# DanielQ-51/cudapathtracer

Measured on AMD Instinct MI355X. Metric: Mray/s, higher is better.
Workload: dtype f32; 1 GPU; cornell_1920x1080_1024spp_depth8_mis; spp=1024, max_depth=8, integrator=UNIDIRECTIONAL (MIS), variant=megakernel, seed=103033, triangles=36, bvh_nodes=31

## Files before the change

### cudapathtracer_amd/csrc/pt_megakernel.h

```cpp
#pragma once
#include "pt_path.h"
#include "pt_params.h"

namespace pt {

PT_DEV void wave_add_total(unsigned long long* totals, int k, uint32_t v) {
    unsigned long long s = v;
    for (int off = 32; off > 0; off >>= 1) s += __shfl_down(s, off, 64);
    if ((threadIdx.x & 63) == 0 && s) atomicAdd(&totals[k], s);
}

extern __shared__ __attribute__((aligned(16))) unsigned char pt_smem[];

PT_DEV SceneCache stage_scene_cache(const DeviceScene& S, int cacheNodes, int cacheTris, int attrOff = 0, int nA = 0, int nM = 0, int nL = 0) {
    typedef __attribute__((address_space(3))) f4v lds_f4;
    lds_f4* dstN = (lds_f4*)pt_smem;
    lds_f4* dstT = dstN + cacheNodes * 4;
    const f4v* srcN = reinterpret_cast<const f4v*>(S.nodes);
    const f4v* srcT = reinterpret_cast<const f4v*>(S.tris);
    for (int i = threadIdx.x; i < cacheNodes * 4; i += blockDim.x) dstN[i] = srcN[i];
    for (int i = threadIdx.x; i < cacheTris * 3; i += blockDim.x) dstT[i] = srcT[i];
    if (attrOff > 0) {
        lds_f4* dA = (lds_f4*)(pt_smem + attrOff);
        lds_f4* dM = dA + nA * 5;
// ... 252 lines not shown
            PT_STAMP(2);
            const int nBusy = __builtin_popcountll(__ballot((rs.flags & kRayBusy) != 0));
            if (nBusy == 0) break;
            trace_resume<COUNT, STACKN, ONCHIP, NOLEAF, TRISEL>(S, SC, st, rs, ps.o, ps.d, (nBusy * P.refillKeep) >> 4, thr, h, c, Keep{P.nodeKeep, P.triKeep});
            PT_STAMP(1);
            continue;
        }
#ifdef PT_STAMPS
        occ[0] += 64; occ[1] += __builtin_popcountll(__ballot((ps.flags & kInPath) != 0 || (samplesLeft > 0 && !stopStarting)));
#endif
        const uint32_t flagsIn = ps.flags;
        if (DEFER) apply_pending<NOLEAF, ARMS>(ps, thr, acc);
        if constexpr (MOMENTS && DEFER) landed_by_apply(flagsIn);
        if (ps.flags & kInPath) {
            bool done = path_bounce<INTEG, COUNT, DEFER, SIMPLE, LEAN, NOLEAF, LTRI, ARMS>(S, ps, ms, h, P.maxDepth, P.useMIS, shadowSync, c, LTRI ? P.lightTri8 : 0ull);
            if (!done) done = path_exhausted<INTEG>(ps, P.maxDepth);
            if (done) { path_finish(ps, acc, DEFER); if constexpr (MOMENTS) landed_by_finish(); }
        }
        PT_STAMP(2);
        while (!(ps.flags & kInPath) && samplesLeft > 0 && !stopStarting) {
            samplesLeft--;
            path_begin<COUNT, ARMS>(P.cam, ps, ms, PT_PX, PT_PY, c);
            if (path_exhausted<INTEG>(ps, P.maxDepth)) { path_finish(ps, acc, DEFER); if constexpr (MOMENTS) landed_by_finish(); }
        }
        if constexpr (ARMS) { if (ps.flags & kDirRaw) ps.d = normalize(ps.d); }
        const bool hasExt = (ps.flags & kInPath) != 0;
        const bool hasShadow = DEFER && (ps.flags & kShadowPending) != 0;
        PT_STAMP(0);
#ifdef PT_STAMPS
        occ[2] += __builtin_popcountll(__ballot(hasExt)); occ[3] += __builtin_popcountll(__ballot(hasShadow));
#endif
        if (__ballot(hasExt || hasShadow) == 0ull) break;
        if constexpr (DEFER && FLAT) {
            trace_pair_flat<STACKN, ARMS>(S, SC, st, hasShadow, ps.so, ps.sd, ps.smaxt, LTRI ? (ps.flags & kLightTriMask) >> kLightTriShift : 0u, hasExt, ps.o, ps.d, thr, h, c, P.cacheNodes, P.leaves, P.nLeaves);
        }
        else if constexpr (FLAT) {
            trace_closest_flat<STACKN, FLATW>(S, SC, hasExt, ps.o, ps.d, 999999.0f, st, h, c, P.cacheNodes, P.leaves, P.nLeaves);
        }
        else if (hasExt) trace_closest<COUNT, STACKN, ONCHIP, CULL>(S, SC, ps.o, ps.d, 999999.0f, st, h, c, Keep{P.nodeKeep, P.triKeep});
        PT_STAMP(1);
    }

    if (lpt) {
        if (lane == 0) { atomicAdd(&P.queue[4], -myRem); atomicAdd(&P.queue[5], -1); }
        __builtin_amdgcn_s_setprio(0);
    }
#ifdef PT_STAMPS
    if (P.totals && lane == 0) {
        for (int k = 0; k < 3; k++) atomicAdd(&P.totals[8 + k], stamp[k]);
        atomicAdd(&P.totals[14], stamp[3]);
        const unsigned long long wall1 = wall_clock64();
        atomicAdd(&P.totals[11], wall1 - wall0);
        atomicMax(&P.totals[12], ~wall0);
        atomicMax(&P.totals[13], wall1);
        if (!COUNT) {
            atomicAdd(&P.totals[0], occ[2]); atomicAdd(&P.totals[1], occ[3]);
            atomicAdd(&P.totals[7], occ[1]); atomicAdd(&P.totals[15], occ[0]);
        }
    }
#endif
    if (inImage) {
        uint32_t* o = (uint32_t*)(P.out + (size_t)lt * 64 + lane);
        state_store(o, __float_as_uint(acc.x), shared); state_store(o + 1, __float_as_uint(acc.y), shared);
        state_store(o + 2, __float_as_uint(acc.z), shared);
    }
    {
        uint32_t* r = P.rng + (size_t)lt * 384 + lane;
// ... 88 lines not shown
```

### cudapathtracer_amd/csrc/pt_plan.h

```cpp
#pragma once
#include "pt_params.h"

namespace pt {

struct Options {
    int variant = 0;
    int cull = 0;
    int schedMask = 31;
    int sliceAlways = 1;
    int sliceIters = 512;
    int lptPrio = 2;
    int persistent = 1;
    int queueTimeoutMs = 30000;
    int onchipOk = 1;
    bool wavesHbmOk = true;
    bool wavesHbmForce = false;
    int nodeKeep = 10, triKeep = 8;
    int refill = 1, refillKeep = 6;
    bool refillKeepSet = false;
    int flatWanted = 1, simpleWanted = 1, leanWanted = 1;
    int leafBoxes = 1;
    int flat2Wanted = 1;
    int wfWideWg = 1;
    int momentsFused = 0;
};
struct Facts {
    DeviceScene ds{};
    int stackNeed = 0, nInternal = 0, cacheNodes = 0, cacheTris = 0, nTrisPacked = 0, nMats = 0, nLightsPacked = 0;
    int nLeaves = 0;
    unsigned long long lightTri8 = 0ull;
    bool armless = false;
    bool noLeafTris = false;
    bool simpleOk = false;
    bool leanOk = false;
    bool flatOk = false;
};

int scene_onchip_wg(const Facts& F, const Options& O);
bool scene_onchip(const Facts& F, const Options& O);
bool hbm_kernel_pays(const Facts& F, const Options& O, int numCU, bool simple, long long tiles);

struct LaunchAsk { int integrator; bool count; int useMIS; int live; };
struct LaunchPlan {
    int onchipWg;
    bool hbm, cull, refill;
    int flat;
    bool simple, lean;
    bool simpleTimed, timedHbm;
};
LaunchPlan plan_launch(const Facts& F, const Options& O, int numCU, const LaunchAsk& ask);
KParams plan_selectors(const LaunchPlan& plan);

struct LaunchSizes { int spillEntries, blocks, queueCap; };
LaunchSizes size_launch(const Facts& F, const Options& O, int numCU, const LaunchAsk& ask, const TileSpan& t, bool listed,
                        const LaunchPlan& plan, const MkRow& row, KParams& P);

}
```

### cudapathtracer_amd/csrc/pt_plan.hip

```cpp
#include <algorithm>

#include "../../include/pt_api.h"
#include "pt_plan.h"

namespace pt {

int scene_onchip_wg(const Facts& F, const Options& O) {
    if (!O.onchipOk || F.nTrisPacked <= 0 || F.ds.stackSpill != 0) return 0;
    const size_t geom = (size_t)F.nInternal * 64 + (size_t)F.nTrisPacked * 48, rec = attr_cache_bytes(F.nTrisPacked, F.nMats, F.nLightsPacked);
    const size_t perWave = (size_t)kStackFlat2Rows * 256 + (F.simpleOk && O.simpleWanted ? 0 : (size_t)kMediumMax * 64);
    for (int wg = 4; wg <= 16; wg *= 2)
        if (geom <= (size_t)kCacheBytes * (wg / 4) && (kAttrCacheBytes == 0 || rec <= (size_t)kAttrCacheBytes * (wg / 4)) &&
            geom + rec + (size_t)wg * perWave <= (size_t)160 * 1024 * wg / 16) return wg;
    return 0;
}
bool scene_onchip(const Facts& F, const Options& O) { return scene_onchip_wg(F, O) > 0; }
bool hbm_kernel_pays(const Facts& F, const Options& O, int numCU, bool simple, long long tiles) {
    if (scene_onchip(F, O) || !O.wavesHbmOk) return false;
    const long long slots = (long long)numCU * 4 * (simple ? kWavesHbmSimple : kWavesHbm);
    return O.wavesHbmForce || tiles * 4 >= slots * (simple ? 3 : 5);
}

LaunchPlan plan_launch(const Facts& F, const Options& O, int numCU, const LaunchAsk& ask) {
    LaunchPlan p = {};
// ... 14 lines not shown
    p.lean = F.leanOk && O.leanWanted && !F.armless && !p.simple && !ask.count && !p.cull && (p.flat == 3 || (!onchip && p.refill));
    return p;
}

KParams plan_selectors(const LaunchPlan& plan) {
    KParams P = {};
    P.onchip = plan.onchipWg > 0 ? 1 : 0;
    P.hbm = plan.hbm ? 1 : 0;
    P.cull = plan.cull ? 1 : 0;
    P.refill = plan.refill ? 1 : 0;
    P.flat = plan.flat;
    P.simple = plan.simple ? 1 : 0;
    P.lean = plan.lean ? 1 : 0;
    return P;
}

LaunchSizes size_launch(const Facts& F, const Options& O, int numCU, const LaunchAsk& ask, const TileSpan& t, bool listed,
                        const LaunchPlan& plan, const MkRow& row, KParams& P) {
    const bool onchip = plan.onchipWg > 0;
    LaunchSizes z = {};
    z.spillEntries = plan.hbm ? std::max(0, F.stackNeed - row.f.stackEntries) : F.ds.stackSpill;
    P.wgWaves = row.f.wgWaves ? row.f.wgWaves : (onchip ? plan.onchipWg : 4);
    P.wavesPerSimd = row.f.wavesPerSimd;
    z.blocks = megakernel_blocks(t.count, P.wgWaves);
    P.S = F.ds;
    P.S.stackSpill = z.spillEntries;
    P.useMIS = ask.useMIS;
    P.tileFirst = t.first; P.tileStride = t.stride; P.tileCount = t.count; P.tilesX = t.tilesX;
    P.cacheNodes = F.cacheNodes; P.cacheTris = F.cacheTris;
    P.lightTri8 = F.lightTri8;
    if (onchip) { P.cacheNodes = F.nInternal; P.cacheTris = F.nTrisPacked; }
    if (onchip && kAttrCacheBytes > 0) { P.cacheAttrs = F.nTrisPacked; P.cacheMats = F.nMats; P.cacheLights = F.nLightsPacked; }
    if (onchip && kAttrCacheBytes > 0 && F.flatOk && O.leafBoxes && F.nLeaves > 0) P.nLeaves = F.nLeaves;
    if (plan.hbm && F.cacheTris == 0) P.cacheNodes = std::min(F.nInternal, (plan.simple ? kCacheBytesHbmSimple : kCacheBytesHbm) / 64);
    P.gnodeFrom = P.cacheNodes;
    if (ask.count && !onchip && F.cacheTris == 0) {
        P.gnodeFrom = plan.timedHbm ? std::min(F.nInternal, (plan.simpleTimed ? kCacheBytesHbmSimple : kCacheBytesHbm) / 64) : F.cacheNodes;
    }
    P.refillKeep = (plan.hbm || O.refillKeepSet) ? O.refillKeep : kRefillKeepSmall;
    P.nodeKeep = O.nodeKeep; P.triKeep = O.triKeep;
    P.lptPrio = O.lptPrio; P.sliceIters = O.sliceIters; P.schedMask = O.schedMask; P.sliceAlways = O.sliceAlways ? 1 : 0;
    P.queueTimeout = (unsigned long long)O.queueTimeoutMs * 100000ull;
    if (O.persistent || listed) {
        z.queueCap = 256;
        while (z.queueCap < t.count) z.queueCap <<= 1;
        P.queueMask = z.queueCap - 1;
        P.gridBlocks = numCU * P.wavesPerSimd * 4 / P.wgWaves;
    }
    return z;
}

}
```

### cudapathtracer_amd/csrc/pt_render.hip

```cpp
#include "pt_host.h"

using namespace pt;

namespace pt {

int resolve_tiles(int w, int h, const pt_tile_range* tiles, TileSpan& t) {
    if (w <= 0 || h <= 0) return fail(-1, "bad image size %dx%d", w, h);
    t.tilesX = (w + 7) / 8;
    int total = t.tilesX * ((h + 7) / 8);
    if (!tiles) { t.first = 0; t.stride = 1; t.count = total; return 0; }
    t.first = tiles->first; t.stride = tiles->stride; t.count = tiles->count;
    if (t.count < 0 || t.stride < 1 || t.first < 0) return fail(-1, "bad tile range {first %d, stride %d, count %d}", t.first, t.stride, t.count);
    if (t.count > 0 && (long long)t.first + (long long)(t.count - 1) * t.stride >= total)
        return fail(-1, "tile range {first %d, stride %d, count %d} exceeds the %d tiles of a %dx%d image", t.first, t.stride, t.count, total, w, h);
    return 0;
}

CamK cam_to_kernel(const pt_camera& c) {
    CamK k;
    k.origin = V3{c.cameraOrigin.x, c.cameraOrigin.y, c.cameraOrigin.z};
    k.forward = V3{c.forward.x, c.forward.y, c.forward.z};
    k.right = V3{c.right.x, c.right.y, c.right.z};
    k.up = V3{c.up.x, c.up.y, c.up.z};
    k.w = c.w; k.h = c.h; k.aperture = c.aperture; k.focalDist = c.focalDist; k.fovScale = c.fovScale; k.jitter = c.antiAliasJitterDist;
// ... 78 lines not shown
    HIP_OK(hipEventRecord(s->dev.ev1, rq.stream));
    s->last.evPending = true;
    return 0;
}

static int render_tiles(pt_scene* s, RenderRequest& rq) {
    const TileSpan& t = rq.t;
    if (t.count == 0) return 0;
    if (rq.fused && s->opt.variant == 1) return 0;
    const int live = rq.list ? rq.live : t.count;
    if (rq.list && (rq.count || s->opt.variant != 0 || t.first != 0 || t.stride != 1 || live < 0 || live > t.count)) return fail(-1, "render_tiles: bad tile list");
    if (int r = s->work.rng.ensure((size_t)t.count * 384 * sizeof(uint32_t))) return r;
    if (!rq.continueStreams) HIP_OK(launch_rng_init((const uint32_t*)s->data.jump.p, rq.seed, rq.w, rq.h, t, (uint32_t*)s->work.rng.p, rq.stream));
    if (rq.fused) rq.seeded = !rq.continueStreams;
    if (s->opt.variant == 1) return render_tiles_wavefront(s, rq);

    const LaunchAsk ask = {rq.integrator, rq.count, rq.useMIS, live};
    const LaunchPlan plan = plan_launch(s->facts, s->opt, s->dev.numCU, ask);
    KParams P = plan_selectors(plan);
    const MkRow* row = megakernel_choose(rq.integrator, rq.count, true, P, false);
    if (!row) return fail(-1, "render_tiles: no megakernel is built for this launch");
    const LaunchSizes z = size_launch(s->facts, s->opt, s->dev.numCU, ask, t, rq.list != nullptr, plan, *row, P);

    if (z.spillEntries > 0)
        if (int r = s->work.spill.ensure((size_t)z.blocks * P.wgWaves * z.spillEntries * 64 * sizeof(int32_t))) return r;
    if (z.queueCap > 0) {
        if (int r = s->work.queue.ensure((size_t)(kQueueHeader + 2 * z.queueCap) * sizeof(int))) return r;
        if (int r = s->work.left.ensure((size_t)t.count * 64 * sizeof(int))) return r;
        P.queue = (int*)s->work.queue.p; P.left = (int*)s->work.left.p;
    }
    P.cam = cam_to_kernel(*rq.cam);
    P.w = rq.w; P.h = rq.h; P.spp = rq.spp; P.maxDepth = rq.maxDepth;
    if (P.nLeaves > 0) P.leaves = (const PLeaf*)s->geo.leaves.p;
    P.rng = (uint32_t*)s->work.rng.p; P.out = (float4*)rq.d_tiles; P.pixCounters = rq.d_pixcnt;
    P.totals = rq.count ? (unsigned long long*)s->data.totals.p : nullptr;
#ifdef PT_STAMPS
    P.totals = (unsigned long long*)s->data.totals.p;
#endif
    P.spill = z.spillEntries > 0 ? (int32_t*)s->work.spill.p : nullptr;

    s->last.lean = P.lean; s->last.refill = P.refill; s->last.hbm = P.hbm;
    s->last.flat = (P.flat && !rq.count) ? 1 : 0;
    s->last.simple = (P.simple && !rq.count) ? 1 : 0;
    s->last.flat2 = (P.flat == 3) ? 1 : 0;
    s->last.leafTable = (P.flat && !rq.count && P.nLeaves > 0) ? 1 : 0;
    s->last.queued = P.queue != nullptr;
    s->last.tiles = t.count;
    s->last.pushed = live;

    MomentsK M = {nullptr, nullptr, 0, 0.0f};
    if (rq.fused) {
        row = megakernel_choose(rq.integrator, rq.count, true, P, true);
        if (!row || (row->key & kMkBuiltOnly)) return 0;
        M.P = rq.P; M.Q = rq.Q; M.c = rq.c; M.rc = 1.0f / (float)rq.c;
        rq.launched = true;
    }
    HIP_OK(hipEventRecord(s->dev.ev0, rq.stream));
    HIP_OK(launch_megakernel(*row, P, live, rq.list, rq.stream, rq.fused ? &M : nullptr));
    HIP_OK(hipEventRecord(s->dev.ev1, rq.stream));
    s->last.evPending = true;
    return 0;
}

int pt_render_tiles_device(pt_scene* s, const pt_camera* cam, int w, int h, int spp, int maxDepth, int integrator, int useMIS,
                           uint64_t seed, const pt_tile_range* tiles, void* d_tile_rgba, int count_work, void* stream) {
    if (int r = check_render_args(s, cam, spp, integrator)) return r;
// ... 355 lines not shown
```

### cudapathtracer_amd/csrc/pt_scene.hip

```cpp
#include <chrono>
#include <cmath>

#include "pt_host.h"
#include "pt_bvh_build.h"
#include "xorwow_host.h"

using namespace pt;

static_assert(sizeof(pt_bvh_node) == 48 && sizeof(pt_triangle) == 80 && sizeof(pt_material) == 176 && sizeof(pt_camera) == 112,
              "boundary structs must keep the reference's CUDA layouts (SURVEY.md Appendix A)");
static_assert(offsetof(pt_triangle, emission) == 48 && offsetof(pt_triangle, lightInd) == 64, "Triangle layout");
static_assert(offsetof(pt_material, type) == 32 && offsetof(pt_material, albedo) == 48 && offsetof(pt_material, eta) == 80 &&
              offsetof(pt_material, ior) == 112 && offsetof(pt_material, isSpecular) == 128 && offsetof(pt_material, absorption) == 144 &&
              offsetof(pt_material, priority) == 160, "Material layout");
static_assert(offsetof(pt_camera, forward) == 64 && offsetof(pt_camera, fovScale) == 44, "Camera layout");

static double wall_ms() { return std::chrono::duration<double, std::milli>(std::chrono::steady_clock::now().time_since_epoch()).count(); }

static int upload(DevBuf& b, const void* src, size_t bytes) {
    if (int r = b.ensure(std::max<size_t>(bytes, 16))) return r;
    if (bytes) HIP_OK(hipMemcpy(b.p, src, bytes, hipMemcpyHostToDevice));
    return 0;
}

static bool boxes_nested_and_finite(const std::vector<PNode>& pn, int nInternal) {
    for (int i = 0; i < nInternal; i++) {
        const PNode& p = pn[i];
        for (int a = 0; a < 3; a++)
            if (!(std::isfinite(p.lmin[a]) && std::isfinite(p.lmax[a]) && std::isfinite(p.rmin[a]) && std::isfinite(p.rmax[a]))) return false;
        const int32_t ref[2] = {p.left, p.right};
        for (int k = 0; k < 2; k++) {
            if (ref[k] < 0) continue;
            if (ref[k] <= i || ref[k] >= nInternal) return false;
            const PNode& c = pn[ref[k]];
            const float* mn = k == 0 ? p.lmin : p.rmin; const float* mx = k == 0 ? p.lmax : p.rmax;
            for (int a = 0; a < 3; a++)
                if (!(mn[a] <= c.lmin[a] && mn[a] <= c.rmin[a] && mx[a] >= c.lmax[a] && mx[a] >= c.rmax[a])) return false;
        }
    }
    return true;
}

template <class LightIndOf>
static void light_triangles(const PTri* pt, int nT, const PLight* lights, int nLights, int nTriangles, LightIndOf lightIndOf, int32_t* out) {
    for (int i = 0; i < nLights; i++) {
        out[i] = -1;
        const PLight& L = lights[i];
        const float v0[3] = {L.a[0], L.a[1], L.a[2]}, e1[3] = {L.b[0] - L.a[0], L.b[1] - L.a[1], L.b[2] - L.a[2]},
                    e2[3] = {L.c[0] - L.a[0], L.c[1] - L.a[1], L.c[2] - L.a[2]};
        for (int p = 0; p < nT && p < 63; p++) {
            const int idx = (int)(pt[p].idx & 0x7fffffffu);
            if (idx >= nTriangles || lightIndOf(idx) != i) continue;
            if (!memcmp(pt[p].v0, v0, 12) && !memcmp(pt[p].e1, e1, 12) && !memcmp(pt[p].e2, e2, 12)) { out[i] = p; break; }
        }
    }
}
static void light_triangles(const PTri* pt, int nT, const pt_scene_desc* d, int32_t* out) {
    std::vector<PLight> L((size_t)std::max(d->n_lights, 1));
    std::vector<uint8_t> bad((size_t)std::max(d->n_lights, 1), 0);
    for (int i = 0; i < d->n_lights; i++) {
        const pt_triangle& t = d->lights[i];
        L[i] = PLight{};
        if (t.aInd < 0 || t.aInd >= d->n_positions || t.bInd < 0 || t.bInd >= d->n_positions || t.cInd < 0 || t.cInd >= d->n_positions) { bad[i] = 1; continue; }
        const pt_float4 a = d->positions[t.aInd], b = d->positions[t.bInd], c = d->positions[t.cInd];
        L[i].a[0] = a.x; L[i].a[1] = a.y; L[i].a[2] = a.z; L[i].b[0] = b.x; L[i].b[1] = b.y; L[i].b[2] = b.z; L[i].c[0] = c.x; L[i].c[1] = c.y; L[i].c[2] = c.z;
    }
    light_triangles(pt, nT, L.data(), d->n_lights, d->n_triangles, [&](int idx) { const int li = d->triangles[idx].lightInd; return (li >= 0 && li < d->n_lights && bad[li]) ? -1 : li; }, out);
}

static int pack_materials(const pt_material* materials, int nMats, int nTexels, const char* fn, std::vector<PMat>& mats, std::vector<uint32_t>& matClass) {
    mats.resize((size_t)nMats); matClass.resize((size_t)nMats);
    std::memset(mats.data(), 0, mats.size() * sizeof(PMat));
    for (int i = 0; i < nMats; i++) {
// ... 83 lines not shown
    if ((size_t)nInternal * 64 + (size_t)nT * 48 <= (size_t)kCacheBytes) { s->facts.cacheNodes = nInternal; s->facts.cacheTris = nT; }
    else { s->facts.cacheNodes = std::min(nInternal, kCacheBytes / 64); s->facts.cacheTris = 0; }
    s->facts.flatOk = false;
    if (nInternal <= 128 && nT >= 1 && nT <= 128 && scene_onchip_wg(s->facts, s->opt) > 0) {
        std::vector<PNode> pn((size_t)std::max(nInternal, 1));
        std::vector<PTri> pt((size_t)nT);
        if (nInternal > 0) HIP_OK(hipMemcpy(pn.data(), s->geo.nodes.p, (size_t)nInternal * sizeof(PNode), hipMemcpyDeviceToHost));
        HIP_OK(hipMemcpy(pt.data(), s->geo.tris.p, (size_t)nT * sizeof(PTri), hipMemcpyDeviceToHost));
        auto leafCount = [&](int first) {
            int k = first;
            while (k < nT) { uint32_t w; memcpy(&w, (const char*)&pt[k] + 36, 4); k++; if (w & 0x80000000u) return k - first; }
            return 0;
        };
        bool ok = rootRef < 0 ? (~rootRef == 0 && leafCount(0) == nT) : (rootRef == 0);
        std::vector<int> first((size_t)std::max(nInternal, 1), 0);
        for (int i = nInternal - 1; i >= 0 && ok; i--) {
            int32_t* ref = &pn[i].left;
            int firstOf[2] = {0, 0};
            for (int k = 0; k < 2 && ok; k++) {
                if (ref[k] >= 0) {
                    ok = ref[k] > i && ref[k] < nInternal;
                    if (ok) { ref[2 + k] = pn[ref[k]].pad0 + pn[ref[k]].pad1; firstOf[k] = first[ref[k]]; }
                } else {
                    const int f = ~ref[k]; const int cnt = (ref[k] != kRefNone && f < nT) ? leafCount(f) : 0;
                    ok = cnt >= 1; ref[2 + k] = cnt; firstOf[k] = f;
                }
            }
            ok = ok && firstOf[1] == firstOf[0] + ref[2];
            first[i] = firstOf[0];
        }
        if (ok && nInternal > 0) ok = first[0] == 0 && pn[0].pad0 + pn[0].pad1 == nT;
        if (ok && nInternal > 0) HIP_OK(hipMemcpy(s->geo.nodes.p, pn.data(), (size_t)nInternal * sizeof(PNode), hipMemcpyHostToDevice));
        s->facts.flatOk = ok;
        s->facts.nLeaves = 0;
        if (ok && nLights > 0 && haveLights) {
            light_triangles(pt.data(), nT, hostLights, nLights, nLightInd, [&](int idx) { return lightIndOf[idx]; }, lightTri.data());
            for (int i = 0; i < nLights && i < 8; i++) s->facts.lightTri8 |= (uint64_t)(lightTri[i] + 1) << (8 * i);
        }
        if (ok && nInternal > 0 && boxes_nested_and_finite(pn, nInternal)) {
            std::vector<PLeaf> lf;
            for (int i = 0; i < nInternal; i++) {
                const int32_t* ref = &pn[i].left;
                for (int k = 0; k < 2; k++) {
                    if (ref[k] >= 0) continue;
                    PLeaf L;
                    const float* mn = k == 0 ? pn[i].lmin : pn[i].rmin; const float* mx = k == 0 ? pn[i].lmax : pn[i].rmax;
                    for (int a = 0; a < 3; a++) { L.mn[a] = mn[a]; L.mx[a] = mx[a]; }
                    L.first = ~ref[k]; L.count = ref[2 + k];
                    lf.push_back(L);
                }
            }
            if (int r = upload(s->geo.leaves, lf.data(), lf.size() * sizeof(PLeaf))) return r;
            s->facts.nLeaves = (int)lf.size();
        }
    }
    return 0;
}

static pt_float4 pos(const pt_scene_desc* d, int i, const char* what, int tri, bool& ok) {
    if (i < 0 || i >= d->n_positions) { ok = false; fail(-1, "pt_scene_create: triangle %d %s index %d out of range", tri, what, i); return pt_float4{0, 0, 0, 0}; }
    return d->positions[i];
}

static int number_nodes(const pt_bvh_node* bvh, int nN, int nT, std::vector<PNode>& nodes, std::vector<uint8_t>& leafEnd, int& nInternal, int& rootRef) {
    std::vector<int> internalId(nN, -1);
    for (int i = 0; i < nN; i++) {
        const pt_bvh_node& n = bvh[i];
        if (n.primCount > 0) {
            if (n.first < 0 || n.first + n.primCount > nT) return fail(-1, "pt_scene_create: leaf %d range [%d,+%d) out of bounds", i, n.first, n.primCount);
        } else {
            if (n.left < 0 || n.right < 0 || n.left >= nN || n.right >= nN) return fail(-1, "pt_scene_create: internal node %d has child out of range", i);
        }
    }
    {
        std::vector<int> queue;
        if (bvh[0].primCount <= 0) { queue.push_back(0); internalId[0] = nInternal++; }
        for (size_t q = 0; q < queue.size(); q++) {
            const pt_bvh_node& n = bvh[queue[q]];
            for (int c : {n.left, n.right}) {
                if (bvh[c].primCount > 0) continue;
                if (internalId[c] >= 0 || (int)queue.size() >= nN) return fail(-1, "pt_scene_create: BVH is not a tree");
                internalId[c] = nInternal++;
                queue.push_back(c);
            }
        }
    }
// ... 449 lines not shown
```

### cudapathtracer_amd/csrc/pt_trace.h

```cpp
#pragma once
#include "pt_device.h"

namespace pt {

struct Ctr {
    uint32_t raysClosest, raysShadow, pops, boxes, tris, hits, draws, iters;
    uint32_t gnodes;
    uint32_t gnodeFrom;
#ifdef PT_UTIL
    uint32_t u[8];
#endif
};
#ifdef PT_UTIL
#define PT_UTIL_STEP(c, k) do { if (COUNT) { (c).u[(k) + 1]++; const uint64_t e_ = __builtin_amdgcn_ballot_w64(true); \
    if (__builtin_amdgcn_mbcnt_hi((uint32_t)(e_ >> 32), __builtin_amdgcn_mbcnt_lo((uint32_t)e_, 0u)) == 0u) (c).u[k]++; } } while (0)
#else
#define PT_UTIL_STEP(c, k) do {} while (0)
#endif

typedef float f4v __attribute__((ext_vector_type(4)));
PT_DEV int32_t f2i(float f) { return __builtin_bit_cast(int32_t, f); }
PT_DEV uint32_t f2u(float f) { return __builtin_bit_cast(uint32_t, f); }
typedef __attribute__((address_space(3))) int32_t lds_i32;
typedef __attribute__((address_space(3))) const f4v lds_cf4;
// ... 142 lines not shown
    return n;
}
struct TriData { f4v a, b, e; };
template <bool ONCHIP = false>
PT_DEV TriData load_tri(const DeviceScene& S, const SceneCache& C, int32_t i) {
    TriData t;
    if (ONCHIP || C.nTris) {
        lds_cf4* p = C.tris + i * 3;
        t.a = p[0]; t.b = p[1]; t.e = p[2];
    } else {
        const f4v* p = reinterpret_cast<const f4v*>(S.tris + i);
        t.a = p[0]; t.b = p[1]; t.e = p[2];
    }
    return t;
}

struct TriEdges { f4v a, b; float e2z; };
PT_DEV TriEdges load_tri_edges(const SceneCache& C, int32_t i) {
    TriEdges t;
    lds_cf4* p = C.tris + i * 3;
    t.a = p[0]; t.b = p[1];
    t.e2z = *reinterpret_cast<__attribute__((address_space(3))) const float*>(p + 2);
    return t;
}
struct LeafBox { float mnx, mny, mnz, mxx, mxy, mxz; int32_t first, count; };
PT_DEV LeafBox leaf_box(const PLeaf* __restrict__ leaves, int k) {
    typedef __attribute__((address_space(4))) const float konst_f;
    typedef __attribute__((address_space(4))) const int32_t konst_i;
    konst_f* p = (konst_f*)(uintptr_t)(leaves + k);
    LeafBox L;
    L.mnx = p[0]; L.mny = p[1]; L.mnz = p[2]; L.mxx = p[3]; L.mxy = p[4]; L.mxz = p[5];
    L.first = ((konst_i*)p)[6]; L.count = ((konst_i*)p)[7];
    return L;
}

struct Keep { int node, tri; };
PT_DEV int lanes_here() { return __builtin_popcountll(__builtin_amdgcn_ballot_w64(true)); }

template <bool COUNT, int N, bool ONCHIP = false, bool CULL = false>
PT_DEV int32_t descend_node(const NodeData& n, int32_t cur, V3 o, V3 inv, Stack<N>& st, Ctr& c, float cullT = 0.0f);

template <bool COUNT, int N, bool ONCHIP = false, bool CULL = false>
PT_DEV int32_t descend(const DeviceScene& S, const SceneCache& C, int32_t cur, V3 o, V3 inv, Stack<N>& st, Ctr& c, float cullT = 0.0f) {
    const NodeData n = load_node<ONCHIP>(S, C, cur);
    return descend_node<COUNT, N, ONCHIP, CULL>(n, cur, o, inv, st, c, cullT);
}

template <bool COUNT, int N, bool ONCHIP, bool CULL>
PT_DEV int32_t descend_node(const NodeData& n, int32_t cur, V3 o, V3 inv, Stack<N>& st, Ctr& c, float cullT) {
    if (COUNT) { c.pops++; c.boxes += 2; if (!ONCHIP && (uint32_t)cur >= c.gnodeFrom) c.gnodes++; }
    float tL, tR;
    bool hL = slab(n.a.x, n.a.y, n.a.z, n.a.w, n.b.x, n.b.y, o, inv, tL);
    bool hR = slab(n.b.z, n.b.w, n.c.x, n.c.y, n.c.z, n.c.w, o, inv, tR);
    if (CULL) { hL = hL && !(tL > cullT); hR = hR && !(tR > cullT); }
    int32_t left = f2i(n.d.x), right = f2i(n.d.y);
    if (!ONCHIP && !COUNT && !CULL && N == 16) {
        if (__builtin_expect(__builtin_amdgcn_ballot_w64(st.sp >= N - 1) == 0ull, 1)) {
            if (hL && hR) {
                bool leftNear = tL < tR;
                st.template push<true>(leftNear ? right : left);
                return leftNear ? left : right;
            }
            if (hL) return left;
            if (hR) return right;
            return st.sp > 0 ? st.template pop<true>() : kRefNone;
        }
// ... 360 lines not shown
                }
                int32_t ref = S.rootRef;
                int lo = 0;
                while (ref >= 0) {
                    const NodeData nd = load_node<true>(S, C, ref);
                    const int mid = lo + f2i(nd.d.z), hi = mid + f2i(nd.d.w);
                    const Set inL = tied & Set::range(lo, mid - lo), inR = tied & Set::range(mid, hi - mid);
                    bool goLeft = !inR.any();
                    if (inL.any() && inR.any()) {
                        float tL, tR;
                        slab(nd.a.x, nd.a.y, nd.a.z, nd.a.w, nd.b.x, nd.b.y, o, inv, tL);
                        slab(nd.b.z, nd.b.w, nd.c.x, nd.c.y, nd.c.z, nd.c.w, o, inv, tR);
                        goLeft = tL < tR;
                    }
                    ref = goLeft ? f2i(nd.d.x) : f2i(nd.d.y);
                    if (!goLeft) lo = mid;
                    tied = goLeft ? inL : inR;
                }
                win = tied.first();
            }
            const TriData q = load_tri<true>(S, C, win);
            float t, u, v;
            moller_trumbore(v3(q.a.x, q.a.y, q.a.z), v3(q.a.w, q.b.x, q.b.y), v3(q.b.z, q.b.w, q.e.x), o, d, t, u, v);
            hit.t = t; hit.u = u; hit.v = v;
            hit.tri = (int32_t)(f2u(q.e.y) & 0x7fffffffu);
            hit.material = f2i(q.e.z);
        }
    }
    wave_lds_sync();
}

template <int N, bool ARMS = false>
PT_DEV void trace_pair_flat(const DeviceScene& S, const SceneCache& C, Stack<N>& st, bool hasShadow, V3 so, V3 sd, float smaxt, uint32_t ltri1,
                            bool hasExt, V3 eo, V3 ed, V3& thr, Hit& hit, Ctr& c, int nInternal, const PLeaf* __restrict__ leaves = nullptr, int nLeaves = 0) {
    static_assert(N >= 24, "the scratch layout needs 24 x 64 words of the wave's stack area");
    typedef __attribute__((address_space(3))) unsigned long long lds_u64;
    const int lane = (int)(threadIdx.x & 63u);
    lds_i32* Wd = st.lds - lane;
    typedef __attribute__((address_space(3))) f4v lds_f4;
    constexpr int kMax = 8 * 128, kKeyA = ARMS ? 8 * 128 : 9 * 128, kKeyB = kKeyA + 256, kPre = kKeyA;
    static_assert(kKeyB + (ARMS ? 256 : 128) == 24 * 64 && (ARMS || kMax + 128 == kKeyA), "records, (bounds,) first minima, second minima: 24 rows of 64 words");
    lds_f4* Rec = (lds_f4*)Wd;
    V3 invE, invS;
    if constexpr (ARMS) { invE = inv3_uniform(ed, hasExt); invS = inv3_uniform(sd, hasShadow); }
    else { invE = inv3(ed); invS = inv3(sd); }
    uint64_t tmE = 0ull, tmS = 0ull;
    if (S.rootRef < 0) { const uint64_t all = ~0ull >> (64 - S.nTris); tmE = hasExt ? all : 0ull; tmS = hasShadow ? all : 0ull; }
    else if (nLeaves > 0 && __builtin_amdgcn_ballot_w64((hasExt && !inv_is_regular(invE)) || (hasShadow && !inv_is_regular(invS))) == 0ull) {
        _Pragma("unroll 2")
        for (int k = 0; k < nLeaves; ++k) {
            const LeafBox L = leaf_box(leaves, k);
            const bool eH = slab_hit(L.mnx, L.mny, L.mnz, L.mxx, L.mxy, L.mxz, eo, invE);
            const bool sH = slab_hit(L.mnx, L.mny, L.mnz, L.mxx, L.mxy, L.mxz, so, invS);
            const uint64_t m = ((1ull << (uint32_t)L.count) - 1ull) << (uint32_t)L.first;
            tmE |= eH ? m : 0ull; tmS |= sH ? m : 0ull;
        }
        tmE = hasExt ? tmE : 0ull; tmS = hasShadow ? tmS : 0ull;
    } else {
        uint64_t visE = hasExt ? 1ull << (uint32_t)S.rootRef : 0ull, visS = hasShadow ? 1ull << (uint32_t)S.rootRef : 0ull;
        for (int i = 0; i < nInternal; ++i) {
            const bool vE = ((visE >> i) & 1ull) != 0ull, vS = ((visS >> i) & 1ull) != 0ull;
            if (__builtin_amdgcn_ballot_w64(vE || vS) == 0ull) continue;
            const NodeData n = load_node<true>(S, C, i);
            float t0, t1;
            const bool eL = slab(n.a.x, n.a.y, n.a.z, n.a.w, n.b.x, n.b.y, eo, invE, t0) && vE;
            const bool eR = slab(n.b.z, n.b.w, n.c.x, n.c.y, n.c.z, n.c.w, eo, invE, t1) && vE;
            const bool sL = slab(n.a.x, n.a.y, n.a.z, n.a.w, n.b.x, n.b.y, so, invS, t0) && vS;
            const bool sR = slab(n.b.z, n.b.w, n.c.x, n.c.y, n.c.z, n.c.w, so, invS, t1) && vS;
            const int32_t left = __builtin_amdgcn_readfirstlane(f2i(n.d.x)), right = __builtin_amdgcn_readfirstlane(f2i(n.d.y));
            const int32_t cntL = __builtin_amdgcn_readfirstlane(f2i(n.d.z)), cntR = __builtin_amdgcn_readfirstlane(f2i(n.d.w));
            const uint64_t bL = left >= 0 ? 1ull << (uint32_t)left : (~0ull >> (64 - cntL)) << (uint32_t)(~left);
            const uint64_t bR = right >= 0 ? 1ull << (uint32_t)right : (~0ull >> (64 - cntR)) << (uint32_t)(~right);
            if (left >= 0) { visE |= eL ? bL : 0ull; visS |= sL ? bL : 0ull; } else { tmE |= eL ? bL : 0ull; tmS |= sL ? bL : 0ull; }
            if (right >= 0) { visE |= eR ? bR : 0ull; visS |= sR ? bR : 0ull; } else { tmE |= eR ? bR : 0ull; tmS |= sR ? bR : 0ull; }
        }
    }
    tmS &= ~((1ull << ltri1) >> 1);
    auto scan = [&](int v, int& total) {
        v += __builtin_amdgcn_update_dpp(0, v, 0x111, 0xf, 0xf, true);
        v += __builtin_amdgcn_update_dpp(0, v, 0x112, 0xf, 0xf, true);
        v += __builtin_amdgcn_update_dpp(0, v, 0x114, 0xf, 0xf, true);
        v += __builtin_amdgcn_update_dpp(0, v, 0x118, 0xf, 0xf, true);
        const int r0 = __builtin_amdgcn_readlane(v, 15), r1 = __builtin_amdgcn_readlane(v, 31), r2 = __builtin_amdgcn_readlane(v, 47);
        v += (lane >= 16 ? r0 : 0) + (lane >= 32 ? r1 : 0) + (lane >= 48 ? r2 : 0);
        total = __builtin_amdgcn_readlane(v, 63);
        return v;
    };
    auto below = [&](uint64_t m) {
// ... 317 lines not shown
```

Baseline: 31990 Mray/s.

## Dedupe leaf boxes into grouped box table for flat pair tracing

Builds a host-side box table that merges leaf boxes with identical bounds into one box carrying a 64-bit triangle mask. It then groups boxes that share the same slab on the best axis and rotates coordinates so that axis comes first. In the ARMS flat-pair path, the shared-axis slab is computed once per group per ray, and each box only tests the remaining two axes. This cuts the number of slab tests in the leaf prefilter, at the cost of extra indirection, a packed parameter in pad0/pad1, and an ARMS-only code path.

Result: faster. 33140 Mray/s, median of 6 (+3.6%).

```diff
diff --git a/cudapathtracer_amd/csrc/pt_box_table.h b/cudapathtracer_amd/csrc/pt_box_table.h
--- /dev/null
+++ b/cudapathtracer_amd/csrc/pt_box_table.h
@@ -0,0 +1,103 @@
+#pragma once
+#include <cmath>
+#include <cstring>
+#include <vector>
+
+#include "pt_device.h"
+
+namespace pt {
+
+inline bool boxes_nested_and_finite(const std::vector<PNode>& pn, int nInternal) {
+    for (int i = 0; i < nInternal; i++) {
+        const PNode& p = pn[i];
+        for (int a = 0; a < 3; a++)
+            if (!(std::isfinite(p.lmin[a]) && std::isfinite(p.lmax[a]) && std::isfinite(p.rmin[a]) && std::isfinite(p.rmax[a]))) return false;
+        const int32_t ref[2] = {p.left, p.right};
+        for (int k = 0; k < 2; k++) {
+            if (ref[k] < 0) continue;
+            if (ref[k] <= i || ref[k] >= nInternal) return false;
+            const PNode& c = pn[ref[k]];
+            const float* mn = k == 0 ? p.lmin : p.rmin; const float* mx = k == 0 ? p.lmax : p.rmax;
+            for (int a = 0; a < 3; a++)
+                if (!(mn[a] <= c.lmin[a] && mn[a] <= c.rmin[a] && mx[a] >= c.lmax[a] && mx[a] >= c.rmax[a])) return false;
+        }
+    }
+    return true;
+}
+
+inline std::vector<PLeaf> build_leaf_table(const std::vector<PNode>& pn, int nInternal) {
+    std::vector<PLeaf> lf;
+    for (int i = 0; i < nInternal; i++) {
+        const int32_t* ref = &pn[i].left;
+        for (int k = 0; k < 2; k++) {
+            if (ref[k] >= 0) continue;
+            PLeaf L;
+            const float* mn = k == 0 ? pn[i].lmin : pn[i].rmin; const float* mx = k == 0 ? pn[i].lmax : pn[i].rmax;
+            for (int a = 0; a < 3; a++) { L.mn[a] = mn[a]; L.mx[a] = mx[a]; }
+            L.first = ~ref[k]; L.count = ref[2 + k];
+            lf.push_back(L);
+        }
+    }
+    return lf;
+}
+
+struct __attribute__((aligned(16))) PBox {
+    float mn[3], mx[3];
+    uint32_t maskLo, maskHi;
+};
+static_assert(sizeof(PBox) == sizeof(PLeaf), "the box table follows the leaf table in one buffer, and the leaf loop reads either as eight dwords");
+
+inline std::vector<PBox> build_box_table(const std::vector<PLeaf>& leaves, int nTris) {
+    std::vector<PBox> bx;
+    if (nTris > 64) return bx;
+    for (const PLeaf& L : leaves) {
+        if (L.first < 0 || L.count < 1 || L.count > 64 || L.first > 64 - L.count) return std::vector<PBox>();
+        const uint64_t m = (L.count == 64 ? ~0ull : (1ull << L.count) - 1ull) << L.first;
+        size_t k = 0;
+        while (k < bx.size() && (std::memcmp(bx[k].mn, L.mn, 12) || std::memcmp(bx[k].mx, L.mx, 12))) k++;
+        if (k == bx.size()) {
+            PBox B;
+            for (int a = 0; a < 3; a++) { B.mn[a] = L.mn[a]; B.mx[a] = L.mx[a]; }
+            B.maskLo = 0u; B.maskHi = 0u;
+            bx.push_back(B);
+        }
+        bx[k].maskLo |= (uint32_t)m; bx[k].maskHi |= (uint32_t)(m >> 32);
+    }
+    return bx;
+}
+
+struct BoxGroups { int axis = 0, nGroups = 0; };
+inline BoxGroups group_box_table(std::vector<PBox>& bx) {
+    BoxGroups G;
+    if (bx.empty()) return G;
+    auto same = [&](const PBox& a, const PBox& b, int ax) { return !std::memcmp(&a.mn[ax], &b.mn[ax], 4) && !std::memcmp(&a.mx[ax], &b.mx[ax], 4); };
+    std::vector<int> best;
+    for (int ax = 0; ax < 3; ax++) {
+        std::vector<int> grp(bx.size());
+        std::vector<size_t> rep;
+        for (size_t k = 0; k < bx.size(); k++) {
+            size_t g = 0;
+            while (g < rep.size() && !same(bx[rep[g]], bx[k], ax)) g++;
+            if (g == rep.size()) rep.push_back(k);
+            grp[k] = (int)g;
+        }
+        if (ax == 0 || (int)rep.size() < G.nGroups) { G.axis = ax; G.nGroups = (int)rep.size(); best = grp; }
+    }
+    std::vector<PBox> out, heads;
+    for (int g = 0; g < G.nGroups; g++) {
+        PBox H{};
+        for (size_t k = 0; k < bx.size(); k++) {
+            if (best[k] != g) continue;
+            PBox B = bx[k];
+            for (int a = 0; a < 3; a++) { B.mn[a] = bx[k].mn[(G.axis + a) % 3]; B.mx[a] = bx[k].mx[(G.axis + a) % 3]; }
+            H.mn[0] = B.mn[0]; H.mx[0] = B.mx[0]; H.maskLo++;
+            out.push_back(B);
+        }
+        heads.push_back(H);
+    }
+    out.insert(out.end(), heads.begin(), heads.end());
+    bx.swap(out);
+    return G;
+}
+
+}
diff --git a/cudapathtracer_amd/csrc/pt_megakernel.h b/cudapathtracer_amd/csrc/pt_megakernel.h
--- a/cudapathtracer_amd/csrc/pt_megakernel.h
+++ b/cudapathtracer_amd/csrc/pt_megakernel.h
@@ -308,7 +308,8 @@
 #endif
         if (__ballot(hasExt || hasShadow) == 0ull) break;
         if constexpr (DEFER && FLAT) {
-            trace_pair_flat<STACKN, ARMS>(S, SC, st, hasShadow, ps.so, ps.sd, ps.smaxt, LTRI ? (ps.flags & kLightTriMask) >> kLightTriShift : 0u, hasExt, ps.o, ps.d, thr, h, c, P.cacheNodes, P.leaves, P.nLeaves);
+            trace_pair_flat<STACKN, ARMS>(S, SC, st, hasShadow, ps.so, ps.sd, ps.smaxt, LTRI ? (ps.flags & kLightTriMask) >> kLightTriShift : 0u, hasExt, ps.o, ps.d, thr, h, c, P.cacheNodes, P.leaves, P.nLeaves,
+                                          ARMS ? P.pad1 : nullptr, ARMS ? P.pad0 : 0);
         }
         else if constexpr (FLAT) {
             trace_closest_flat<STACKN, FLATW>(S, SC, hasExt, ps.o, ps.d, 999999.0f, st, h, c, P.cacheNodes, P.leaves, P.nLeaves);
diff --git a/cudapathtracer_amd/csrc/pt_plan.h b/cudapathtracer_amd/csrc/pt_plan.h
--- a/cudapathtracer_amd/csrc/pt_plan.h
+++ b/cudapathtracer_amd/csrc/pt_plan.h
@@ -28,6 +28,7 @@
     DeviceScene ds{};
     int stackNeed = 0, nInternal = 0, cacheNodes = 0, cacheTris = 0, nTrisPacked = 0, nMats = 0, nLightsPacked = 0;
     int nLeaves = 0;
+    int nBoxes = 0, nBoxGroups = 0, boxAxis = 0;
     unsigned long long lightTri8 = 0ull;
     bool armless = false;
     bool noLeafTris = false;
diff --git a/cudapathtracer_amd/csrc/pt_plan.hip b/cudapathtracer_amd/csrc/pt_plan.hip
--- a/cudapathtracer_amd/csrc/pt_plan.hip
+++ b/cudapathtracer_amd/csrc/pt_plan.hip
@@ -70,6 +70,7 @@
     if (onchip) { P.cacheNodes = F.nInternal; P.cacheTris = F.nTrisPacked; }
     if (onchip && kAttrCacheBytes > 0) { P.cacheAttrs = F.nTrisPacked; P.cacheMats = F.nMats; P.cacheLights = F.nLightsPacked; }
     if (onchip && kAttrCacheBytes > 0 && F.flatOk && O.leafBoxes && F.nLeaves > 0) P.nLeaves = F.nLeaves;
+    if (P.nLeaves > 0 && plan.flat == 3) P.pad0 = F.nBoxes | (F.nBoxGroups << 8) | (F.boxAxis << 16);
     if (plan.hbm && F.cacheTris == 0) P.cacheNodes = std::min(F.nInternal, (plan.simple ? kCacheBytesHbmSimple : kCacheBytesHbm) / 64);
     P.gnodeFrom = P.cacheNodes;
     if (ask.count && !onchip && F.cacheTris == 0) {
diff --git a/cudapathtracer_amd/csrc/pt_render.hip b/cudapathtracer_amd/csrc/pt_render.hip
--- a/cudapathtracer_amd/csrc/pt_render.hip
+++ b/cudapathtracer_amd/csrc/pt_render.hip
@@ -134,6 +134,7 @@
     P.cam = cam_to_kernel(*rq.cam);
     P.w = rq.w; P.h = rq.h; P.spp = rq.spp; P.maxDepth = rq.maxDepth;
     if (P.nLeaves > 0) P.leaves = (const PLeaf*)s->geo.leaves.p;
+    if (P.pad0 > 0) P.pad1 = P.leaves + s->facts.nLeaves;
     P.rng = (uint32_t*)s->work.rng.p; P.out = (float4*)rq.d_tiles; P.pixCounters = rq.d_pixcnt;
     P.totals = rq.count ? (unsigned long long*)s->data.totals.p : nullptr;
 #ifdef PT_STAMPS
diff --git a/cudapathtracer_amd/csrc/pt_scene.hip b/cudapathtracer_amd/csrc/pt_scene.hip
--- a/cudapathtracer_amd/csrc/pt_scene.hip
+++ b/cudapathtracer_amd/csrc/pt_scene.hip
@@ -3,6 +3,7 @@
 
 #include "pt_host.h"
 #include "pt_bvh_build.h"
+#include "pt_box_table.h"
 #include "xorwow_host.h"
 
 using namespace pt;
@@ -21,24 +22,6 @@
     if (int r = b.ensure(std::max<size_t>(bytes, 16))) return r;
     if (bytes) HIP_OK(hipMemcpy(b.p, src, bytes, hipMemcpyHostToDevice));
     return 0;
-}
-
-static bool boxes_nested_and_finite(const std::vector<PNode>& pn, int nInternal) {
-    for (int i = 0; i < nInternal; i++) {
-        const PNode& p = pn[i];
-        for (int a = 0; a < 3; a++)
-            if (!(std::isfinite(p.lmin[a]) && std::isfinite(p.lmax[a]) && std::isfinite(p.rmin[a]) && std::isfinite(p.rmax[a]))) return false;
-        const int32_t ref[2] = {p.left, p.right};
-        for (int k = 0; k < 2; k++) {
-            if (ref[k] < 0) continue;
-            if (ref[k] <= i || ref[k] >= nInternal) return false;
-            const PNode& c = pn[ref[k]];
-            const float* mn = k == 0 ? p.lmin : p.rmin; const float* mx = k == 0 ? p.lmax : p.rmax;
-            for (int a = 0; a < 3; a++)
-                if (!(mn[a] <= c.lmin[a] && mn[a] <= c.rmin[a] && mx[a] >= c.lmax[a] && mx[a] >= c.rmax[a])) return false;
-        }
-    }
-    return true;
 }
 
 template <class LightIndOf>
@@ -188,26 +171,21 @@
         if (ok && nInternal > 0) ok = first[0] == 0 && pn[0].pad0 + pn[0].pad1 == nT;
         if (ok && nInternal > 0) HIP_OK(hipMemcpy(s->geo.nodes.p, pn.data(), (size_t)nInternal * sizeof(PNode), hipMemcpyHostToDevice));
         s->facts.flatOk = ok;
-        s->facts.nLeaves = 0;
+        s->facts.nLeaves = 0; s->facts.nBoxes = 0; s->facts.nBoxGroups = 0; s->facts.boxAxis = 0;
         if (ok && nLights > 0 && haveLights) {
             light_triangles(pt.data(), nT, hostLights, nLights, nLightInd, [&](int idx) { return lightIndOf[idx]; }, lightTri.data());
             for (int i = 0; i < nLights && i < 8; i++) s->facts.lightTri8 |= (uint64_t)(lightTri[i] + 1) << (8 * i);
         }
         if (ok && nInternal > 0 && boxes_nested_and_finite(pn, nInternal)) {
-            std::vector<PLeaf> lf;
-            for (int i = 0; i < nInternal; i++) {
-                const int32_t* ref = &pn[i].left;
-                for (int k = 0; k < 2; k++) {
-                    if (ref[k] >= 0) continue;
-                    PLeaf L;
-                    const float* mn = k == 0 ? pn[i].lmin : pn[i].rmin; const float* mx = k == 0 ? pn[i].lmax : pn[i].rmax;
-                    for (int a = 0; a < 3; a++) { L.mn[a] = mn[a]; L.mx[a] = mx[a]; }
-                    L.first = ~ref[k]; L.count = ref[2 + k];
-                    lf.push_back(L);
-                }
-            }
+            std::vector<PLeaf> lf = build_leaf_table(pn, nInternal);
+            std::vector<PBox> bx = build_box_table(lf, nT);
+            const int nBoxes = (int)bx.size();
+            const BoxGroups G = group_box_table(bx);
+            const size_t nLeaves = lf.size();
+            lf.resize(nLeaves + bx.size());
+            if (!bx.empty()) memcpy((void*)(lf.data() + nLeaves), bx.data(), bx.size() * sizeof(PBox));
             if (int r = upload(s->geo.leaves, lf.data(), lf.size() * sizeof(PLeaf))) return r;
-            s->facts.nLeaves = (int)lf.size();
+            s->facts.nLeaves = (int)nLeaves; s->facts.nBoxes = nBoxes; s->facts.nBoxGroups = G.nGroups; s->facts.boxAxis = G.axis;
         }
     }
     return 0;
diff --git a/cudapathtracer_amd/csrc/pt_trace.h b/cudapathtracer_amd/csrc/pt_trace.h
--- a/cudapathtracer_amd/csrc/pt_trace.h
+++ b/cudapathtracer_amd/csrc/pt_trace.h
@@ -198,6 +198,18 @@
     L.mnx = p[0]; L.mny = p[1]; L.mnz = p[2]; L.mxx = p[3]; L.mxy = p[4]; L.mxz = p[5];
     L.first = ((konst_i*)p)[6]; L.count = ((konst_i*)p)[7];
     return L;
+}
+struct PairBox { float mng, mnu, mnv, mxg, mxu, mxv; uint64_t mask; };
+PT_DEV PairBox pair_box(const void* __restrict__ boxes, int k) {
+    typedef uint32_t u8v __attribute__((ext_vector_type(8)));
+    typedef __attribute__((address_space(4))) const u8v konst_rec;
+    const u8v r = *((konst_rec*)(uintptr_t)boxes + k);
+    const uint32_t w0 = r[0], w1 = r[1], w2 = r[2], w3 = r[3], w4 = r[4], w5 = r[5];
+    PairBox B;
+    B.mng = __builtin_bit_cast(float, w0); B.mnu = __builtin_bit_cast(float, w1); B.mnv = __builtin_bit_cast(float, w2);
+    B.mxg = __builtin_bit_cast(float, w3); B.mxu = __builtin_bit_cast(float, w4); B.mxv = __builtin_bit_cast(float, w5);
+    B.mask = (uint64_t)r[6] | ((uint64_t)r[7] << 32);
+    return B;
 }
 
 struct Keep { int node, tri; };
@@ -624,7 +636,8 @@
 
 template <int N, bool ARMS = false>
 PT_DEV void trace_pair_flat(const DeviceScene& S, const SceneCache& C, Stack<N>& st, bool hasShadow, V3 so, V3 sd, float smaxt, uint32_t ltri1,
-                            bool hasExt, V3 eo, V3 ed, V3& thr, Hit& hit, Ctr& c, int nInternal, const PLeaf* __restrict__ leaves = nullptr, int nLeaves = 0) {
+                            bool hasExt, V3 eo, V3 ed, V3& thr, Hit& hit, Ctr& c, int nInternal, const PLeaf* __restrict__ leaves = nullptr, int nLeaves = 0,
+                            const void* __restrict__ boxes = nullptr, int nBoxes = 0) {
     static_assert(N >= 24, "the scratch layout needs 24 x 64 words of the wave's stack area");
     typedef __attribute__((address_space(3))) unsigned long long lds_u64;
     const int lane = (int)(threadIdx.x & 63u);
@@ -638,7 +651,34 @@
     else { invE = inv3(ed); invS = inv3(sd); }
     uint64_t tmE = 0ull, tmS = 0ull;
     if (S.rootRef < 0) { const uint64_t all = ~0ull >> (64 - S.nTris); tmE = hasExt ? all : 0ull; tmS = hasShadow ? all : 0ull; }
-    else if (nLeaves > 0 && __builtin_amdgcn_ballot_w64((hasExt && !inv_is_regular(invE)) || (hasShadow && !inv_is_regular(invS))) == 0ull) {
+    else if ((ARMS ? nBoxes : nLeaves) > 0 && __builtin_amdgcn_ballot_w64((hasExt && !inv_is_regular(invE)) || (hasShadow && !inv_is_regular(invS))) == 0ull) {
+        if constexpr (ARMS) {
+            const int nB = nBoxes & 255, nG = (nBoxes >> 8) & 255, axis = nBoxes >> 16;
+            auto rot = [&](V3 a) { return axis == 0 ? a : (axis == 1 ? v3(a.y, a.z, a.x) : v3(a.z, a.x, a.y)); };
+            const V3 oE = rot(eo), iE = rot(invE), oS = rot(so), iS = rot(invS);
+            auto uv_hit = [](float gmn, float gmx, const PairBox& B, V3 o, V3 inv) {
+                const float tu1 = (B.mnu - o.y) * inv.y, tu2 = (B.mxu - o.y) * inv.y;
+                float tmn = fmaxf_(gmn, fminf_(tu1, tu2)), tmx = fminf_(gmx, fmaxf_(tu1, tu2));
+                const float tv1 = (B.mnv - o.z) * inv.z, tv2 = (B.mxv - o.z) * inv.z;
+                tmn = fmaxf_(tmn, fminf_(tv1, tv2)); tmx = fminf_(tmx, fmaxf_(tv1, tv2));
+                return tmx >= tmn;
+            };
+            int k = 0;
+            for (int g = 0; g < nG; ++g) {
+                const PairBox H = pair_box(boxes, nB + g);
+                const float e1 = (H.mng - oE.x) * iE.x, e2 = (H.mxg - oE.x) * iE.x;
+                const float gmnE = fmaxf_(1.401298464e-45f, fminf_(e1, e2)), gmxE = fminf_(1e30f, fmaxf_(e1, e2));
+                const float s1 = (H.mng - oS.x) * iS.x, s2 = (H.mxg - oS.x) * iS.x;
+                const float gmnS = fmaxf_(1.401298464e-45f, fminf_(s1, s2)), gmxS = fminf_(1e30f, fmaxf_(s1, s2));
+                const int end = k + (int)(uint32_t)H.mask;
+                do {
+                    const PairBox B = pair_box(boxes, k);
+                    const bool eH = uv_hit(gmnE, gmxE, B, oE, iE);
+                    const bool sH = uv_hit(gmnS, gmxS, B, oS, iS);
+                    tmE |= eH ? B.mask : 0ull; tmS |= sH ? B.mask : 0ull;
+                } while (++k < end);
+            }
+        } else {
         _Pragma("unroll 2")
         for (int k = 0; k < nLeaves; ++k) {
             const LeafBox L = leaf_box(leaves, k);
@@ -646,6 +686,7 @@
             const bool sH = slab_hit(L.mnx, L.mny, L.mnz, L.mxx, L.mxy, L.mxz, so, invS);
             const uint64_t m = ((1ull << (uint32_t)L.count) - 1ull) << (uint32_t)L.first;
             tmE |= eH ? m : 0ull; tmS |= sH ? m : 0ull;
+        }
         }
         tmE = hasExt ? tmE : 0ull; tmS = hasShadow ? tmS : 0ull;
     } else {
```
